# acerbilab/gpyreg

Hardware: AMD Instinct MI355X
Metric: GP-fits/sec (NLL+grad, N=4096 D=10) (higher is better)
Workload: dtype f64

## Files before the change

gpyreg_amd/csrc/gemm.h:

```cpp
#pragma once
#include "common.h"

#include <type_traits>

namespace gpc {

template <typename T>
constexpr int BKT_v = sizeof(T) == 4 ? 32 : 16;
template <typename T>
constexpr bool MM_SWZ = sizeof(T) == 4;
template <typename T>
constexpr int LDQ_v = MM_SWZ<T> ? BKT_v<T> : BKT_v<T> + 1;
constexpr int ldp_of(int BT) { return BT + 16; }
template <typename T>
constexpr int opsz_of(int BT) {
  return BKT_v<T> * (BT + 16) > BT * LDQ_v<T> ? BKT_v<T> * (BT + 16) : BT * LDQ_v<T>;
}

enum { KLO_ZERO = 0, KLO_ROW = 1, KLO_COL = 2 };
enum { KHI_FULL = 0, KHI_ROW = 1, KHI_COL = 2 };

struct GemmArgs {
  const void* A;
  const void* B;
  void* C;
  long long sA, sB, sC;
  int lda, ldb, ldc;
  int M, N, K;
  double alpha;
  int beta;
  int klo, khi, lower_only;
  int tiles_m, tiles_n;
  int flags = 0;
  const unsigned short* rsv = nullptr;
  int* ctr = nullptr;
  int ntiles = 0, batch = 0;
  double* colsq = nullptr;
  const double* ep_w = nullptr;
  long long ep_sw = 0;
  const double* ep_alpha = nullptr;
};
inline int g_gemm_flags = 8 | 16;

template <typename T, bool KM, int BT, int NT>
__device__ __forceinline__ unsigned stage_toff(int ld, int t) {
  constexpr int VEC = MM<T>::VEC;
  if constexpr (!KM) {
    constexpr int TPR = BKT_v<T> / VEC;
    return (unsigned)(t / TPR) * (unsigned)ld + (unsigned)((t % TPR) * VEC);
  } else {
    constexpr int VPR = BT / VEC;
    return (unsigned)(t / VPR) * (unsigned)ld + (unsigned)((t % VPR) * VEC);
  }
}
template <typename T, bool KM, int BT, int NT>
__device__ __forceinline__ size_t stage_pstride(int ld) {
// ... 107 lines not shown
  const int total = gx * gy, per = total >> 3;
  const int L = by * gx + bx;
  if (L < (per << 3)) {
    const int wk = (L & 7) * per + (L >> 3);
    bx = wk % gx;
    by = wk / gx;
  }
}

#ifdef GPC_TILE_TRACE
__device__ unsigned long long g_tile_trace[2][4];
#define TILE_TS(k) do { if (HO && threadIdx.x == 0) { const long long _n = wall_clock64(); atomicAdd(&g_tile_trace[BT == 64][k], (unsigned long long)(_n - _ts)); _ts = _n; } } while (0)
#else
#define TILE_TS(k) do { } while (0)
#endif
template <typename T, bool AKM, bool BKM, int BT, int NW, int HO = 0, int EPI = 0, int BTN = BT>
__device__ __forceinline__ void gemm_tile(const GemmArgs& g, const int bx, const int by, T* __restrict__ smem) {
#ifdef GPC_TILE_TRACE
  long long _ts = wall_clock64();
  if (HO && threadIdx.x == 0) atomicAdd(&g_tile_trace[BT == 64][3], 1ull);
#endif
  using acc_t = typename MM<T>::acc_t;
  using vec_t = typename MM<T>::vec_t;
  constexpr int NT = 64 * NW;
  constexpr int NVA = (BT * BKT_v<T>) / (NT * MM<T>::VEC), NVB = (BTN * BKT_v<T>) / (NT * MM<T>::VEC);
  constexpr int OPSZA = opsz_of<T>(BT), OPSZB = opsz_of<T>(BTN), STG = OPSZA + OPSZB;
  constexpr int WCOLS = NW / 2;
  constexpr int WTM = BT / 2;
  constexpr int WTN = BTN / WCOLS;
  constexpr int MRM = WTM / 16, MRN = WTN / 16;
  static_assert(NVA >= 1 && NVB >= 1 && MRM >= 1 && MRN >= 1, "tile shape");
  const int t = threadIdx.x;
  const int lane = t & 63, w = t >> 6, wr = w / WCOLS, wc = w % WCOLS;

  static_assert(BTN == BT || BT == 2 * BTN, "lower tiles of a rectangular launch: two tile columns per tile row");
  int ti, tj;
  tile_of_bx<BTN == BT>(g.klo, g.khi, g.lower_only, g.tiles_m, g.tiles_n, bx, ti, tj);
  const int m0 = ti * BT, n0 = tj * BTN;
  const int m128 = (m0 / TILE) * TILE, n128 = (n0 / TILE) * TILE;
  int k0 = g.klo == KLO_ROW ? m128 : (g.klo == KLO_COL ? n128 : 0);
  int k1 = g.khi == KHI_ROW ? m128 + TILE : (g.khi == KHI_COL ? n128 + TILE : g.K);
  if (k1 > g.K) k1 = g.K;
  const int nk = (k1 - k0) / BKT_v<T>;

  const T* __restrict__ A = reinterpret_cast<const T*>(g.A) + (size_t)by * g.sA;
  const T* __restrict__ B = reinterpret_cast<const T*>(g.B) + (size_t)by * g.sB;
  T* __restrict__ C = reinterpret_cast<T*>(g.C) + (size_t)by * g.sC;

// ... 38 lines not shown
    };
    constexpr int AUX = HO == 1 ? 16 : 0;
    g2r<T, AKM, BT, NT, AUX>(ra, rsa, ua, psa, toa);
    g2r<T, BKM, BTN, NT, AUX>(rb, rsb, ub, psb, tob);
    r2s<T, AKM, BT, NT>(smem, ra, t);
    r2s<T, BKM, BTN, NT>(smem + OPSZA, rb, t);
    next_slab();
    g2r<T, AKM, BT, NT, AUX>(ra, rsa, ua, psa, toa);
    g2r<T, BKM, BTN, NT, AUX>(rb, rsb, ub, psb, tob);
    __syncthreads();
    TILE_TS(0);

    T af[2][MRM], bf[2][MRN];
    auto load_frags = [&](int set, const T* a_s, const T* b_s, int kk) {
#pragma unroll
      for (int i = 0; i < MRM; ++i) af[set][i] = frag<T, AKM, BT>(a_s, wr * WTM + i * 16, kk, lane);
#pragma unroll
      for (int j = 0; j < MRN; ++j) bf[set][j] = frag<T, BKM, BTN>(b_s, wc * WTN + j * 16, kk, lane);
    };
    auto mfmas = [&](int set) {
#pragma unroll
      for (int i = 0; i < MRM; ++i)
#pragma unroll
        for (int j = 0; j < MRN; ++j) acc[i][j] = MM<T>::mma(af[set][i], bf[set][j], acc[i][j]);
    };
    constexpr int NMEM = NVA + NVB;
    constexpr int PER = (MRM * MRN) / NMEM;
    constexpr int REM = MRM * MRN - PER * NMEM;
    static_assert(PER >= 1, "interleave pattern");
    constexpr int KS = BKT_v<T> / 4;
    static_assert(KS >= 4 && KS % 2 == 0, "fragment sets alternate per k-step and wrap per slab");
    auto slab = [&](auto cur_c, auto wr_c, auto ld_c) {
      constexpr int CUR = decltype(cur_c)::value;
// ... 28 lines not shown
        g2r<T, BKM, BTN, NT, AUX>(rb, rsb, ub, psb, tob);
      }
      if constexpr (WR) load_frags(0, a_n, a_n + OPSZA, 0);
      mfmas(1);
      if constexpr (WR) __builtin_amdgcn_sched_group_barrier(0x100, MRM + MRN, 0);
#pragma unroll
      for (int q = 0; q < NMEM; ++q) {
        __builtin_amdgcn_sched_group_barrier(0x008, PER, 0);
        if constexpr (LD) __builtin_amdgcn_sched_group_barrier(0x020, 1, 0);
      }
      if constexpr (REM > 0) __builtin_amdgcn_sched_group_barrier(0x008, REM, 0);
    };
    using I0 = std::integral_constant<int, 0>;
    using I1 = std::integral_constant<int, 1>;
    load_frags(0, smem, smem + OPSZA, 0);
    int it = 0;
    for (; it + 3 < nk; it += 2) {
      slab(I0{}, std::true_type{}, std::true_type{});
      slab(I1{}, std::true_type{}, std::true_type{});
      if constexpr (TWO_LEVEL) {
#pragma unroll
        for (int i = 0; i < MRM; ++i)
#pragma unroll
          for (int j = 0; j < MRN; ++j) {
            acc2[i][j] += acc[i][j];
            acc[i][j] = acc_t{0, 0, 0, 0};
          }
      }
    }
    slab(I0{}, std::true_type{}, std::false_type{});
    slab(I1{}, std::false_type{}, std::false_type{});
  }

  TILE_TS(1);
  const T alpha = (T)g.alpha;
  if constexpr (EPI == 1) {
    static_assert(NW == 4 && BT == 128 && BTN == BT, "the reduction is laid out for 2 x 2 waves of 64 x 64");
    double cs[MRN];
#pragma unroll
    for (int j = 0; j < MRN; ++j) {
      double sq = 0.0;
#pragma unroll
      for (int i = 0; i < MRM; ++i)
#pragma unroll
        for (int r = 0; r < 4; ++r) {
          double v;
// ... 65 lines not shown
      for (int j = 0; j < MRN; ++j) red[wr * BT + wc * WTN + j * 16 + (lane & 15)] = cs[j];
    }
    __syncthreads();
    if (t < BT) g.colsq[((size_t)by * g.tiles_m + ti) * (size_t)g.N + n0 + t] = red[t] + red[BT + t];
    __syncthreads();
    return;
  }
#pragma unroll
  for (int i = 0; i < MRM; ++i) {
    T old[MRN][4];
    if (g.beta) {
#pragma unroll
      for (int j = 0; j < MRN; ++j)
#pragma unroll
        for (int r = 0; r < 4; ++r) {
          const int row = m0 + wr * WTM + i * 16 + MM<T>::row_of(lane, r);
          const int col = n0 + wc * WTN + j * 16 + (lane & 15);
          if constexpr (HO == 1)
            old[j][r] = __hip_atomic_load(&C[(size_t)row * g.ldc + col], __ATOMIC_RELAXED, __HIP_MEMORY_SCOPE_AGENT);
          else
            old[j][r] = C[(size_t)row * g.ldc + col];
        }
    }
#pragma unroll
    for (int j = 0; j < MRN; ++j)
#pragma unroll
      for (int r = 0; r < 4; ++r) {
        const int row = m0 + wr * WTM + i * 16 + MM<T>::row_of(lane, r);
        const int col = n0 + wc * WTN + j * 16 + (lane & 15);
        T v;
        if constexpr (TWO_LEVEL)
          v = alpha * (acc[i][j][r] + acc2[i][j][r]);
        else
          v = alpha * acc[i][j][r];
        if (g.beta) v += old[j][r];
        if constexpr (HO)
          __hip_atomic_store(&C[(size_t)row * g.ldc + col], v, __ATOMIC_RELAXED, __HIP_MEMORY_SCOPE_AGENT);
        else
          C[(size_t)row * g.ldc + col] = v;
      }
  }
  TILE_TS(2);
}

template <typename T, bool AKM, bool BKM, int BT, int NW, int EPI = 0, int BTN = BT>
__global__ __launch_bounds__(64 * NW, NW / 2) void gemm_kernel(GemmArgs g) {
  __shared__ __attribute__((aligned(16))) T smem[2 * (opsz_of<T>(BT) + opsz_of<T>(BTN))];
  int bx = blockIdx.x, by = blockIdx.y;
  if ((g.flags & 16) && gridDim.y >= 8) {
    xcd_order((int)gridDim.x, (int)gridDim.y, bx, by);
  }
  gemm_tile<T, AKM, BKM, BT, NW, 0, EPI, BTN>(g, bx, by, smem);
}

template <typename T, bool A1, bool B1, bool A2, bool B2, int BT, int NW>
__global__ __launch_bounds__(64 * NW, NW / 2) void gemm_dual_kernel(GemmArgs g1, GemmArgs g2, int n1) {
  __shared__ __attribute__((aligned(16))) T smem[4 * opsz_of<T>(BT)];
  int bx = blockIdx.x, by = blockIdx.y;
  if ((g1.flags & 16) && gridDim.y >= 8) xcd_order((int)gridDim.x, (int)gridDim.y, bx, by);
  if (bx < n1)
    gemm_tile<T, A1, B1, BT, NW>(g1, bx, by, smem);
  else
    gemm_tile<T, A2, B2, BT, NW>(g2, bx - n1, by, smem);
}

template <typename T, bool AKM, bool BKM, int BT, int NW, int EPI = 0>
__global__ __launch_bounds__(64 * NW, NW / 2) void gemm_persist_kernel(GemmArgs g) {
  __shared__ __attribute__((aligned(16))) T smem[4 * opsz_of<T>(BT)];
  __shared__ int next_tile;
  if (g.rsv && cu_reserve_bail(g.rsv, g.ctr)) return;
  if (!(g.flags & 8)) {
    const int total = g.ntiles * g.batch;
    for (;;) {
      if (threadIdx.x == 0) next_tile = atomicAdd(g.ctr, 1);
      __syncthreads();
      const int idx = __builtin_amdgcn_readfirstlane(next_tile);
      __syncthreads();
      if (idx >= total) break;
      gemm_tile<T, AKM, BKM, BT, NW, 0, EPI>(g, idx / g.batch, idx % g.batch, smem);
    }
    return;
  }
  unsigned xcc;
  asm volatile("s_getreg_b32 %0, hwreg(HW_REG_XCC_ID)" : "=s"(xcc));
  const int q0 = (int)(xcc & (NQ - 1));
  const int nclass = g.batch >= NQ ? 1 : NQ / g.batch;
  for (int a = 0; a < NQ; ++a) {
    const int q = (q0 + a) & (NQ - 1);
    int nsq, cls = 0, smp = q;
    if (g.batch >= NQ) {
      nsq = (g.batch - q + NQ - 1) / NQ;
    } else {
      if (q >= g.batch * nclass) continue;
      nsq = 1;
      smp = q % g.batch;
      cls = q / g.batch;
    }
    if (nsq <= 0) continue;
    const int total = ((g.ntiles - cls + nclass - 1) / nclass) * nsq;
    for (;;) {
      if (threadIdx.x == 0) next_tile = atomicAdd(g.ctr + q, 1);
      __syncthreads();
      const int idx = __builtin_amdgcn_readfirstlane(next_tile);
      __syncthreads();
      if (idx >= total) break;
      const int ntq = total / nsq;
      const int sq = idx / ntq, tq = idx - sq * ntq;
      gemm_tile<T, AKM, BKM, BT, NW, 0, EPI>(g, cls + tq * nclass, smp + NQ * sq, smem);
    }
  }
}

inline int queue_nclass(int batch) { return batch >= NQ ? 1 : NQ / batch; }
inline int queue_of(int batch, int nclass, int q, int& cls, int& smp) {
  int nsq;
  cls = 0;
  smp = q;
  if (batch >= NQ) {
    nsq = (batch - q + NQ - 1) / NQ;
  } else {
    if (q >= batch * nclass) return 0;
    nsq = 1;
    smp = q % batch;
    cls = q / batch;
  }
  return nsq;
}
inline int queue_total(int ntiles, int nclass, int cls, int nsq) { return ((ntiles - cls + nclass - 1) / nclass) * nsq; }
inline void queue_item(int total, int nsq, int nclass, int cls, int smp, int idx, int& tile, int& sample) {
  const int ntq = total / nsq;
  const int sq = idx / ntq, tq = idx - sq * ntq;
  tile = cls + tq * nclass;
  sample = smp + NQ * sq;
}
inline void flat_queue_item(int batch, int idx, int& tile, int& sample) {
  tile = idx / batch;
  sample = idx % batch;
}

inline int g_persist_spare = 0;
inline long long g_gemm_launches = 0;
inline int g_block_slots = 512;
template <typename T, int BT, int NW>
inline hipError_t launch_gemm_bt(hipStream_t st, GemmArgs g, bool akm, bool bkm, int batch, int* ctr = nullptr,
                                 const unsigned short* reserve = nullptr) {
  const int tm = g.M / BT, tn = g.N / BT;
  g.tiles_m = tm;
  g.tiles_n = tn;
  g.flags = g_gemm_flags;
  const int ntiles = g.lower_only ? tm * (tm + 1) / 2 : tm * tn;
  if (ntiles <= 0 || batch <= 0) return hipSuccess;
  ++g_gemm_launches;
  g.ntiles = ntiles;
  g.batch = batch;
  g.ctr = ctr;
  const unsigned dyn = 0u;
  const int cap = (BT == 128 ? g_block_slots : 2 * g_block_slots) - g_persist_spare;
  g.rsv = reserve;
  if (ctr && (BT == 128 || reserve) && cap > 0 && ((long long)ntiles * batch > cap || reserve)) {
    dim3 grid(reserve ? (BT == 128 ? cap + 96 : cap) : cap), block(64 * NW);
    if (!akm && !bkm)
      hipLaunchKernelGGL((gemm_persist_kernel<T, false, false, BT, NW>), grid, block, dyn, st, g);
    else if (!akm && bkm)
      hipLaunchKernelGGL((gemm_persist_kernel<T, false, true, BT, NW>), grid, block, dyn, st, g);
    else if (akm && bkm)
      hipLaunchKernelGGL((gemm_persist_kernel<T, true, true, BT, NW>), grid, block, dyn, st, g);
    else
      hipLaunchKernelGGL((gemm_persist_kernel<T, true, false, BT, NW>), grid, block, dyn, st, g);
    return hipGetLastError();
  }
  dim3 grid(ntiles, batch), block(64 * NW);
  if (!akm && !bkm)
    hipLaunchKernelGGL((gemm_kernel<T, false, false, BT, NW>), grid, block, dyn, st, g);
  else if (!akm && bkm)
    hipLaunchKernelGGL((gemm_kernel<T, false, true, BT, NW>), grid, block, dyn, st, g);
  else if (akm && bkm)
    hipLaunchKernelGGL((gemm_kernel<T, true, true, BT, NW>), grid, block, dyn, st, g);
  else
    hipLaunchKernelGGL((gemm_kernel<T, true, false, BT, NW>), grid, block, dyn, st, g);
  return hipGetLastError();
}

#ifdef GPC_EXPERIMENTS
template <typename T>
inline hipError_t launch_gemm_rect(hipStream_t st, GemmArgs g, bool akm, bool bkm, int batch) {
  constexpr int BT = 128, BTN = 64;
// ... 39 lines not shown
  else if (akm && bkm)
    hipLaunchKernelGGL((gemm_kernel<T, true, true, BT, 8>), grid, block, 0, st, g);
  else
    hipLaunchKernelGGL((gemm_kernel<T, true, false, BT, 8>), grid, block, 0, st, g);
  return hipGetLastError();
}
inline int g_rect_min_blocks = 0;
inline int g_rect_mode = 0;

#else
constexpr int g_rect_min_blocks = 0;
#endif

inline int g_small_launch_blocks = 1100;
inline bool g_dual_launch = true;
template <typename T>
inline hipError_t launch_gemm(hipStream_t st, GemmArgs g, bool akm, bool bkm, int batch, int force_bt = 0,
                             int* ctr = nullptr, const unsigned short* reserve = nullptr, int reserved_small_bt = 128) {
  const int tm = g.M / TILE, tn = g.N / TILE;
  const long long blocks128 = (long long)(g.lower_only ? tm * (tm + 1) / 2 : tm * tn) * batch;
  const bool small = force_bt ? (force_bt == 64) : (blocks128 < g_small_launch_blocks);
#ifdef GPC_EXPERIMENTS
  if ((force_bt == 12864 || (!force_bt && small && g_rect_min_blocks > 0 && blocks128 >= g_rect_min_blocks)) && !(reserve && ctr))
    return (g_rect_mode == 1 && force_bt != 12864) ? launch_gemm_w8<T>(st, g, akm, bkm, batch) : launch_gemm_rect<T>(st, g, akm, bkm, batch);
#endif
  if (small && !(reserve && ctr)) return launch_gemm_bt<T, 64, 4>(st, g, akm, bkm, batch);
#ifdef GPC_EXPERIMENTS
  if (small && reserved_small_bt == 64) return launch_gemm_bt<T, 64, 4>(st, g, akm, bkm, batch, ctr, reserve);
#endif
  return launch_gemm_bt<T, 128, 4>(st, g, akm, bkm, batch, ctr, ctr ? reserve : nullptr);
// ... 83 lines not shown
```

gpyreg_amd/csrc/gpcore.hip:

```cpp
#include "../../include/gpcore.h"

#include <algorithm>
#include <atomic>
#include <chrono>
#include <cmath>
#include <cstdlib>
#include <cstring>
#include <memory>
#include <mutex>

#include "blas1.h"
#include "block_append.h"
#include "common.h"
#include "covfun.h"
#include "cv.h"
#include "cvgrad.h"
#include "draw.h"
#include "gemm.h"
#include "gradpost.h"
#include "hess.h"
#include "hypgrad.h"
#include "nll_hess.h"
#include "leaf.h"
#include "lookahead.h"
// ... 3987 lines not shown
              {rb, cb, p.ldb, p.off_b, p.s_b, p.size_b, true},
              {p.M, p.N, p.ldc, p.off_c, p.s_c, p.size_c, false}};
  for (const Op& o : ops) {
    if (o.ld < o.cols || o.off < 0 || o.stride < 0 || o.size <= 0 || o.size > CAP || o.ld > CAP || o.stride > CAP)
      return "leading dimension below the extent, or a negative / oversized offset, stride or allocation";
    const long long span = (o.rows - 1) * o.ld + o.cols;
    if (o.off + (batch - 1) * o.stride + span > o.size) return "an operand reaches past its allocation";
    if (o.staged && (o.ld % vec || o.off % vec || o.stride % vec))
      return "lda, ldb and the offsets and strides of A and B must be multiples of the 16-byte vector";
    if (!o.staged && batch > 1 && o.stride < span) return "the C blocks of two samples overlap";
  }
  return nullptr;
}

template <typename T>
int debug_gemm_form_impl(gpc_ctx* c, int form, int tile, int batch, int flags, int block_slots,
                         const gpc_gemm_product* const* prods, int nprod, const double* ep_w, long long ep_sw,
                         const double* ep_alpha, double* colsq, int* counters, int* available) {
  HookMem mem;
  GemmGlobalsGuard guard;
  if (flags >= 0) gpc::g_gemm_flags = flags;
  if (block_slots > 0) {
    gpc::g_block_slots = block_slots;
    gpc::g_persist_spare = 0;
  }
  const unsigned short* rsv = nullptr;
  if (form == GPC_FORM_PERSIST_RESERVED) {
    rsv = ctx_reserve_tbl(c);
    if (!rsv) {
      *available = 0;
      return 0;
// ... 25 lines not shown
    a.C = dC[i] + p.off_c;
    a.sA = p.s_a;
    a.sB = p.s_b;
    a.sC = p.s_c;
    a.lda = p.lda;
    a.ldb = p.ldb;
    a.ldc = p.ldc;
    a.M = p.M;
    a.N = p.N;
    a.K = p.K;
    a.alpha = p.alpha;
    a.beta = p.beta;
    a.klo = p.klo;
    a.khi = p.khi;
    a.lower_only = p.lower_only ? 1 : 0;
  }
  int* ctr = nullptr;
  HIPCHK(c, mem.get(reinterpret_cast<void**>(&ctr), CTR_STRIDE * sizeof(int)));
  HIPCHK(c, hipMemsetAsync(ctr, 0, CTR_STRIDE * sizeof(int), c->st));
  const gpc_gemm_product& p0 = *prods[0];
  const size_t ncolsq = (size_t)batch * (p0.M / TILE) * p0.N;
  double* dcolsq = nullptr;
  if (form == GPC_FORM_COLSQ || form == GPC_FORM_WSQ) {
    HIPCHK(c, mem.get(reinterpret_cast<void**>(&dcolsq), ncolsq * sizeof(double)));
    HIPCHK(c, hipMemsetAsync(dcolsq, 0xff, ncolsq * sizeof(double), c->st));
    g[0].colsq = dcolsq;
  }
  if (form == GPC_FORM_WSQ) {
    double *dw = nullptr, *da = nullptr;
    const size_t nw = (size_t)(batch - 1) * ep_sw + p0.M;
// ... 2454 lines not shown
#ifdef GPC_EXPERIMENTS
constexpr int IS_EXPERIMENTS_BUILD = 1;
#else
constexpr int IS_EXPERIMENTS_BUILD = 0;
#endif
int clamp_to(int lo, int hi, int v) { return std::max(lo, std::min(hi, v)); }
int tile_multiple(int v) { return std::max(TILE, (v / TILE) * TILE); }
int engine_choice(int v) { return v == 1 || v == 2 ? v : 0; }
#define GPC_GET(expr) [](gpc_ctx* c) -> int { (void)c; return (int)(expr); }
#define GPC_SET(stmt) [](gpc_ctx* c, int v) -> int { (void)c; stmt; return 0; }
#define GPC_COUNTER(field) GPC_GET(c->field & 0x7fffffff), nullptr
const Option OPTIONS[] = {
    {"groups", GPC_GET(c->groups), GPC_SET(c->groups = clamp_to(1, gpc_ctx::MAXG, v))},
    {"small_blocks", GPC_GET(gpc::g_small_launch_blocks), GPC_SET(gpc::g_small_launch_blocks = v)},
    {"dual_launch", GPC_GET(gpc::g_dual_launch ? 1 : 0), GPC_SET(gpc::g_dual_launch = v != 0)},
    {"leaf", GPC_GET(gpc::g_leaf_version), GPC_SET(gpc::g_leaf_version = v == 3 ? 3 : 5)},
    {"defer_min", GPC_GET(c->defer_min), GPC_SET(c->defer_min = v)},
    {"defer_reserve", GPC_GET(c->defer_reserve), [](gpc_ctx* c, int v) -> int { return c->defer_reserve = v, build_reserve_table(c); }},
    {"leaf_fault", nullptr, GPC_SET(gpc::g_leaf_fault = v != 0)},
    {"nll_block", GPC_GET(c->nll_block), GPC_SET(c->nll_block = v < 0 ? -1 : (v == 0 ? 0 : tile_multiple(v)))},
    {"solves_beside_lauum", GPC_GET(c->solves_beside_lauum), GPC_SET(c->solves_beside_lauum = v != 0)},
    {"stable", GPC_GET(c->stable), GPC_SET(c->stable = v != 0)},
    {"small_path", GPC_GET(c->small_path), GPC_SET(c->small_path = v != 0)},
    {"check_queues", GPC_GET(c->check_queues), GPC_SET(c->check_queues = v != 0)},
    {"small_poll", GPC_GET(c->small_poll), GPC_SET(c->small_poll = v != 0)},
    {"small_timing", GPC_GET(c->small_timing), GPC_SET(c->small_timing = v != 0)},
    {"small_polled", GPC_COUNTER(small_polled)},
    {"small_synced", GPC_COUNTER(small_synced)},
    {"hess_contract_us", GPC_COUNTER(hess_contract_us)},
    {"nll_hess_gram_us", GPC_COUNTER(nll_hess_gram_us)},
// ... 206 lines not shown
    for (int by = 0; by < batch; ++by)
      for (int bx = 0; bx < ntiles; ++bx) {
        int x = bx, y = by;
        if ((flags & 16) && batch >= 8) xcd_order(ntiles, batch, x, y);
        xcd_items[2 * (by * ntiles + bx)] = x;
        xcd_items[2 * (by * ntiles + bx) + 1] = y;
      }
  }
  return 0;
}

int gpc_debug_gemm_form(gpc_ctx* c, int dtype, int form, int tile, int batch, int flags, int block_slots,
                        const gpc_gemm_product* p1, const gpc_gemm_product* p2, const double* ep_w, long long ep_sw,
                        const double* ep_alpha, double* colsq, int* counters, int* available) {
  if (!c) return -2;
  if (!p1 || !counters || !available || batch <= 0 || batch > 64 || form < GPC_FORM_PLAIN || form > GPC_FORM_WSQ ||
      (tile != 64 && tile != 128) || (dtype != GPC_F64 && dtype != GPC_F32) || flags > 31 || block_slots > 4096)
    FAIL(c, "gpc_debug_gemm_form: bad arguments");
  const int vec = dtype == GPC_F64 ? 2 : 4;
  const gpc_gemm_product* prods[2] = {p1, p2};
  const int nprod = form == GPC_FORM_DUAL ? 2 : 1;
  if (nprod == 2 && !p2) FAIL(c, "gpc_debug_gemm_form: the dual form takes two products");
  for (int i = 0; i < nprod; ++i)
    if (const char* e = form_product_error(*prods[i], batch, vec)) {
      c->err = std::string("gpc_debug_gemm_form: ") + e;
      return -2;
    }
  if (form == GPC_FORM_DUAL && (p1->a_kmajor || p1->b_kmajor || p2->a_kmajor || !p2->b_kmajor))
    FAIL(c, "gpc_debug_gemm_form: the dual launch is m-major x m-major beside m-major x k-major");
  if (form == GPC_FORM_COLSQ && (p1->a_kmajor || !p1->b_kmajor || p1->lower_only || !colsq))
    FAIL(c, "gpc_debug_gemm_form: colsq is m-major x k-major over all tiles and needs the colsq output");
  if (form == GPC_FORM_WSQ && (!p1->a_kmajor || !p1->b_kmajor || p1->lower_only || !colsq || !ep_w || !ep_alpha ||
                               (batch > 1 && ep_sw != 0 && ep_sw < p1->M) || ep_sw < 0 || ep_sw > (1ll << 27)))
    FAIL(c, "gpc_debug_gemm_form: wsq is k-major x k-major over all tiles and needs colsq, ep_w, ep_alpha");
  HIPCHK(c, hipSetDevice(c->device));
  return dtype == GPC_F64 ? debug_gemm_form_impl<double>(c, form, tile, batch, flags, block_slots, prods, nprod, ep_w, ep_sw,
                                                         ep_alpha, colsq, counters, available)
                          : debug_gemm_form_impl<float>(c, form, tile, batch, flags, block_slots, prods, nprod, ep_w, ep_sw,
                                                        ep_alpha, colsq, counters, available);
}

int gpc_debug_leaf(gpc_ctx* c, int dtype, const double* A, double* L, double* W, double* logdet, int* info) {
  return gpc_debug_factor(c, dtype, TILE, A, L, W, nullptr, logdet, info);
}

int gpc_debug_factor(gpc_ctx* c, int dtype, int n, const double* A, double* L, double* W, double* Ainv,
                     double* logdet, int* info) {
  if (!c) return -2;
  if (!A || n <= 0) FAIL(c, "gpc_debug_factor: bad arguments");
  HIPCHK(c, hipSetDevice(c->device));
  return dtype == GPC_F64 ? debug_factor_impl<double>(c, n, A, L, W, Ainv, logdet, info)
                          : debug_factor_impl<float>(c, n, A, L, W, Ainv, logdet, info);
}
// ... 305 lines not shown
```

gpyreg_amd/csrc/plan.h:

```cpp
#pragma once
#include "blas1.h"
#include "gemm.h"
#include "leaf.h"

#include <algorithm>

namespace gpc {

#ifdef GPC_EXPERIMENTS
struct PlanRecorder {
  struct Op {
    int kind;
    GemmArgs g;
    bool akm, bkm;
    int off;
  };
  std::vector<Op> ops;
  bool unsupported = false;
};
#endif

template <typename T>
struct Factor {
#ifdef GPC_EXPERIMENTS
// ... 20 lines not shown
  const unsigned short* reserve = nullptr;
  struct QueueCheck {
    int* slot;
    int ntiles, batch;
  };
  std::vector<QueueCheck>* qlog = nullptr;
#ifdef GPC_EXPERIMENTS
  bool reserve_all = false;
  int reserve_min = 64;
  int reserved_small_bt = 128;
#else
  static constexpr bool reserve_all = false;
  static constexpr int reserve_min = 64, reserved_small_bt = 128;
#endif
  bool dual_launch = g_dual_launch;
  bool stable = false;
  hipEvent_t ev_tail = nullptr;
  int tail_row0 = 1 << 30;
  void need_rows(int hi) {
    if (ev_tail && hi > tail_row0) {
      chk(hipStreamWaitEvent(st, ev_tail, 0));
      ev_tail = nullptr;
    }
  }
  double flops = 0;
  int launches = 0;
  hipError_t err = hipSuccess;

  T* blk(T* base, int r, int c) const { return base + (size_t)r * npad + c; }

// ... 10 lines not shown
    g.M = M;
    g.N = N;
    g.K = K;
    g.alpha = alpha;
    g.beta = beta;
    g.klo = klo;
    g.khi = khi;
    g.lower_only = lower;
    g.tiles_n = N / TILE;
    flops += gemm_flops(g, batch);
    return g;
  }

  void gemm(T* C, long long sC, const T* Aop, long long sAop, const T* Bop, long long sBop, int M,
            int N, int K, bool akm, bool bkm, double alpha, int beta, int klo, int khi, int lower,
            hipStream_t on = nullptr, const unsigned short* rsv = nullptr) {
    GemmArgs g;
    g.A = Aop;
    g.B = Bop;
    g.C = C;
    g.sA = sAop;
    g.sB = sBop;
    g.sC = sC;
    g.lda = g.ldb = g.ldc = npad;
    g.M = M;
    g.N = N;
    g.K = K;
    g.alpha = alpha;
    g.beta = beta;
    g.klo = klo;
    g.khi = khi;
    g.lower_only = lower;
    g.tiles_n = N / TILE;
    flops += gemm_flops(g, batch);
    ++launches;
#ifdef GPC_EXPERIMENTS
    if (rec) {
      rec->ops.push_back({0, g, akm, bkm, 0});
      return;
    }
#endif
    int* slot = nullptr;
    const long long tm = M / TILE, tn = N / TILE;
    const long long blocks128 = (lower ? tm * (tm + 1) / 2 : tm * tn) * batch;
    if (!rsv && reserve_all && reserve && blocks128 >= reserve_min) rsv = reserve;
    const bool persistent = rsv || (blocks128 >= g_small_launch_blocks && blocks128 > g_block_slots - g_persist_spare);
    if (persistent && ctr && ctr_used + CTR_STRIDE <= ctr_cap) {
// ... 22 lines not shown
      }
#endif
      need_rows(off + TILE);
      launch_leaf<T>(st, batch, blk(A, off, off), sA, npad, blk(W, off, off), sW, npad, off, logdet, info,
                     std::max(0, std::min(TILE, nvalid - off)), stable);
      flops += (2.0 / 3.0) * TILE * (double)TILE * TILE * batch;
      ++launches;
      return;
    }
    const int q = n / TILE;
    const int n1 = (q / 2) * TILE, n2 = n - n1;
    const int o1 = off, o2 = off + n1;
    potrf_inv(o1, n1, true, keep_L);
    need_rows(o2 + n2);
    gemm(blk(Tm, o2, o1), sT, blk(A, o2, o1), sA, blk(W, o1, o1), sW, n2, n1, n1, false, false, 1.0,
         0, KLO_ZERO, KHI_COL, 0);
    if (stable) {
      gemm(blk(A, o2, o1), sA, blk(Tm, o2, o1), sT, blk(A, o1, o1), sA, n2, n1, n1, false, false, -1.0, 1, KLO_ZERO,
           KHI_COL, 0);
      gemm(blk(Tm, o2, o1), sT, blk(A, o2, o1), sA, blk(W, o1, o1), sW, n2, n1, n1, false, false, 1.0, 1, KLO_ZERO,
           KHI_COL, 0);
    }
    const bool defer = need_inv && side && defer_min > 0 && n >= defer_min && ev_used + 2 <= nev;
    bool u_done = false;
    {
      GemmArgs gs = make_args(blk(A, o2, o2), sA, blk(Tm, o2, o1), sT, blk(Tm, o2, o1), sT, n2, n2, n1, -1.0, 1,
                              KLO_ZERO, KHI_FULL, 1);
      const long long syrk_tiles = (long long)(n2 / TILE) * (n2 / TILE + 1) / 2 * batch;
      if (need_inv && !defer && dual_launch && !rec && gemm_is_small(gs, batch) && !(reserve_all && syrk_tiles >= reserve_min)) {
        GemmArgs gu = make_args(blk(A, o2, o1), sA, blk(Tm, o2, o1), sT, blk(W, o1, o1), sW, n2, n1, n1, 1.0, 0,
                                KLO_COL, KHI_FULL, 0);
// ... 7 lines not shown
        }
      }
      if (!u_done) {
        flops -= gemm_flops(gs, batch);
        gemm(blk(A, o2, o2), sA, blk(Tm, o2, o1), sT, blk(Tm, o2, o1), sT, n2, n2, n1, false, false, -1.0, 1,
             KLO_ZERO, KHI_FULL, 1);
      }
    }
    hipEvent_t ev_join = nullptr;
    if (defer) {
      hipEvent_t ev_fork = evs[ev_used++];
      ev_join = evs[ev_used++];
      chk(hipEventRecord(ev_fork, st));
      chk(hipStreamWaitEvent(side, ev_fork, 0));
      gemm(blk(A, o2, o1), sA, blk(Tm, o2, o1), sT, blk(W, o1, o1), sW, n2, n1, n1, false, true, 1.0, 0,
           KLO_COL, KHI_FULL, 0, side, reserve);
      chk(hipEventRecord(ev_join, side));
    }
    potrf_inv(o2, n2, need_inv, keep_L);
    if (need_inv) {
      if (defer)
        chk(hipStreamWaitEvent(st, ev_join, 0));
      else if (!u_done)
        gemm(blk(A, o2, o1), sA, blk(Tm, o2, o1), sT, blk(W, o1, o1), sW, n2, n1, n1, false, true, 1.0, 0,
             KLO_COL, KHI_FULL, 0);
      gemm(blk(W, o2, o1), sW, blk(W, o2, o2), sW, blk(A, o2, o1), sA, n2, n1, n2, false, true, -1.0,
           0, KLO_ZERO, KHI_ROW, 0);
    }
#ifdef GPC_EXPERIMENTS
    if (keep_L && rec) rec->unsupported = true;
#endif
    if (keep_L && !rec) {
      dim3 grid((n1 + 64 * MM<T>::VEC - 1) / (64 * MM<T>::VEC), n2 / 32, batch), block(64, 4);
      hipLaunchKernelGGL((rect_copy_kernel<T>), grid, block, 0, st, (const T*)blk(Tm, o2, o1), sT, npad,
                         blk(A, o2, o1), sA, npad, n2, n1);
      ++launches;
    }
  }

  int nll_block = 0;

  void trsm_nll(int r0, int m, int c0, int n) {
// ... 114 lines not shown
        hipLaunchKernelGGL((trmv_kernel<T>), dim3(n / 4, batch), dim3(256), 0, st, (const T*)W, sW, npad,
                           (const double*)r, npad, z, off);
      ++launches;
      return;
    }
    const int q = n / TILE;
    const int n1 = (q / 2) * TILE, n2 = n - n1;
    forward_solve(off, n1, true, r, z);
    hipLaunchKernelGGL((gemv_sub_kernel<T>), dim3(n2 / 4, batch), dim3(256), 0, st, (const T*)Tm, sT, npad,
                       (const double*)z, r, npad, off + n1, off, n1);
    ++launches;
    forward_solve(off + n1, n2, need_inv, r, z);
  }

  void lauum(T* out, long long sOut) {
    gemm(out, sOut, W, sW, W, sW, npad, npad, npad, true, true, 1.0, 0, KLO_ROW, KHI_FULL, 1);
  }
};

}
```

Before: 844.5.

## Skip zero MFMAs inside triangular diagonal blocks of fp64 128-tile GEMMs

Adds a TRI template mode to the fp64 128-tile GEMM. In the k-slabs that cross a triangular operand's diagonal block, each wave issues only the MFMAs for sub-tile rows or columns that can be nonzero. The wave-to-subtile mapping is interleaved so the skipped work is spread evenly across waves. The mode is wired into the trsm, inverse-update and lauum calls, with a runtime toggle that defaults to on. In exchange it adds kernel instantiations, runtime branches in the slab loop, and a changed fragment layout that may cost register or scheduling efficiency.

```diff
diff --git a/gpyreg_amd/csrc/gemm.h b/gpyreg_amd/csrc/gemm.h
--- a/gpyreg_amd/csrc/gemm.h
+++ b/gpyreg_amd/csrc/gemm.h
@@ -19,6 +19,7 @@
 
 enum { KLO_ZERO = 0, KLO_ROW = 1, KLO_COL = 2 };
 enum { KHI_FULL = 0, KHI_ROW = 1, KHI_COL = 2 };
+enum { TRI_NONE = 0, TRI_A_FIRST = 1, TRI_B_FIRST = 2, TRI_B_LAST = 3, TRI_A_LAST = 4 };
 
 struct GemmArgs {
   const void* A;
@@ -32,6 +33,7 @@
   int klo, khi, lower_only;
   int tiles_m, tiles_n;
   int flags = 0;
+  int tri = 0;
   const unsigned short* rsv = nullptr;
   int* ctr = nullptr;
   int ntiles = 0, batch = 0;
@@ -40,6 +42,7 @@
   long long ep_sw = 0;
   const double* ep_alpha = nullptr;
 };
+static_assert(sizeof(GemmArgs) == 168, "tri fills the hole behind flags: the kernel arguments keep their offsets and size");
 inline int g_gemm_flags = 8 | 16;
 
 template <typename T, bool KM, int BT, int NT>
@@ -177,7 +180,7 @@
 #else
 #define TILE_TS(k) do { } while (0)
 #endif
-template <typename T, bool AKM, bool BKM, int BT, int NW, int HO = 0, int EPI = 0, int BTN = BT>
+template <typename T, bool AKM, bool BKM, int BT, int NW, int HO = 0, int EPI = 0, int BTN = BT, int TRI = 0>
 __device__ __forceinline__ void gemm_tile(const GemmArgs& g, const int bx, const int by, T* __restrict__ smem) {
 #ifdef GPC_TILE_TRACE
   long long _ts = wall_clock64();
@@ -193,8 +196,16 @@
   constexpr int WTN = BTN / WCOLS;
   constexpr int MRM = WTM / 16, MRN = WTN / 16;
   static_assert(NVA >= 1 && NVB >= 1 && MRM >= 1 && MRN >= 1, "tile shape");
+  static_assert(TRI == 0 || (sizeof(T) == 8 && BT == 128 && BTN == BT && NW == 4 && HO == 0 && EPI == 0),
+                "triangular blocks: the fp64 128-tile of 2 x 2 waves, stored");
+  static_assert(TRI == 0 || (TRI == TRI_A_FIRST && AKM) || (TRI == TRI_B_FIRST && BKM) || (TRI == TRI_B_LAST && !BKM) ||
+                    (TRI == TRI_A_LAST && !AKM), "the orientation of the triangular operand");
   const int t = threadIdx.x;
   const int lane = t & 63, w = t >> 6, wr = w / WCOLS, wc = w % WCOLS;
+#define GPC_WROW(i) (TRI ? (wr + 2 * (i)) * 16 : wr * WTM + (i) * 16)
+#define GPC_WCOL(j) (TRI ? (wc + 2 * (j)) * 16 : wc * WTN + (j) * 16)
+#define GPC_ROW(o, i) (TRI ? (o) + (wr + 2 * (i)) * 16 : (o) + wr * WTM + (i) * 16)
+#define GPC_COL(o, j) (TRI ? (o) + (wc + 2 * (j)) * 16 : (o) + wc * WTN + (j) * 16)
 
   static_assert(BTN == BT || BT == 2 * BTN, "lower tiles of a rectangular launch: two tile columns per tile row");
   int ti, tj;
@@ -263,9 +274,9 @@
     T af[2][MRM], bf[2][MRN];
     auto load_frags = [&](int set, const T* a_s, const T* b_s, int kk) {
 #pragma unroll
-      for (int i = 0; i < MRM; ++i) af[set][i] = frag<T, AKM, BT>(a_s, wr * WTM + i * 16, kk, lane);
-#pragma unroll
-      for (int j = 0; j < MRN; ++j) bf[set][j] = frag<T, BKM, BTN>(b_s, wc * WTN + j * 16, kk, lane);
+      for (int i = 0; i < MRM; ++i) af[set][i] = frag<T, AKM, BT>(a_s, GPC_WROW(i), kk, lane);
+#pragma unroll
+      for (int j = 0; j < MRN; ++j) bf[set][j] = frag<T, BKM, BTN>(b_s, GPC_WCOL(j), kk, lane);
     };
     auto mfmas = [&](int set) {
 #pragma unroll
@@ -324,22 +335,103 @@
     using I0 = std::integral_constant<int, 0>;
     using I1 = std::integral_constant<int, 1>;
     load_frags(0, smem, smem + OPSZA, 0);
-    int it = 0;
-    for (; it + 3 < nk; it += 2) {
-      slab(I0{}, std::true_type{}, std::true_type{});
-      slab(I1{}, std::true_type{}, std::true_type{});
-      if constexpr (TWO_LEVEL) {
-#pragma unroll
-        for (int i = 0; i < MRM; ++i)
-#pragma unroll
-          for (int j = 0; j < MRN; ++j) {
-            acc2[i][j] += acc[i][j];
-            acc[i][j] = acc_t{0, 0, 0, 0};
+    if constexpr (TRI != 0) {
+      constexpr bool ON_A = TRI == TRI_A_FIRST || TRI == TRI_A_LAST, FIRST = TRI == TRI_A_FIRST || TRI == TRI_B_FIRST;
+      const int wq = __builtin_amdgcn_readfirstlane(ON_A ? wr : wc);
+      auto mfmas_tri = [&](int set, int lo, int hi) {
+        if constexpr (ON_A) {
+#pragma unroll
+          for (int i = 0; i < MRM; ++i)
+            if (i >= lo && i < hi) {
+#pragma unroll
+              for (int j = 0; j < MRN; ++j) acc[i][j] = MM<T>::mma(af[set][i], bf[set][j], acc[i][j]);
+            }
+        } else {
+#pragma unroll
+          for (int j = 0; j < MRN; ++j)
+            if (j >= lo && j < hi) {
+#pragma unroll
+              for (int i = 0; i < MRM; ++i) acc[i][j] = MM<T>::mma(af[set][i], bf[set][j], acc[i][j]);
+            }
+        }
+      };
+      auto slab_tri = [&](auto cur_c, const bool WR, const bool LD, const int lo, const int hi) {
+        constexpr int CUR = decltype(cur_c)::value;
+        const T* a_s = smem + CUR * STG;
+        const T* b_s = a_s + OPSZA;
+        T* a_n = smem + (CUR ^ 1) * STG;
+#pragma unroll
+        for (int ks = 0; ks < KS - 2; ++ks) {
+          load_frags((ks + 1) & 1, a_s, b_s, 4 * (ks + 1));
+          mfmas_tri(ks & 1, lo, hi);
+        }
+        load_frags(1, a_s, b_s, 4 * (KS - 1));
+        if (WR) {
+          r2s<T, AKM, BT, NT>(a_n, ra, t);
+          r2s<T, BKM, BTN, NT>(a_n + OPSZA, rb, t);
+        }
+        mfmas_tri(0, lo, hi);
+        __syncthreads();
+        if (LD) {
+          next_slab();
+          g2r<T, AKM, BT, NT, AUX>(ra, rsa, ua, psa, toa);
+          g2r<T, BKM, BTN, NT, AUX>(rb, rsb, ub, psb, tob);
+        }
+        if (WR) load_frags(0, a_n, a_n + OPSZA, 0);
+        mfmas_tri(1, lo, hi);
+      };
+      auto tri_pair = [&](const int s, const bool more) {
+        int lo[2], hi[2];
+#pragma unroll
+        for (int e = 0; e < 2; ++e) {
+          const int d = s + e - wq;
+          lo[e] = FIRST ? 0 : (d > 0 ? (d + 1) >> 1 : 0);
+          hi[e] = FIRST ? (d >= 0 ? (d >> 1) + 1 : 0) : 4;
+        }
+        slab_tri(I0{}, true, more, lo[0], hi[0]);
+        slab_tri(I1{}, more, more, lo[1], hi[1]);
+      };
+      constexpr int NTRI = TILE / BKT_v<T>;
+      static_assert(MRM == 4 && MRN == 4 && NTRI == 8, "live prefixes and suffixes of four tile-rows over eight slabs");
+      if constexpr (FIRST) {
+#pragma unroll 1
+        for (int s = 0; s < NTRI; s += 2) tri_pair(s, s + 2 < nk);
+        if (nk > NTRI) {
+#pragma unroll 1
+          for (int it = NTRI; it + 3 < nk; it += 2) {
+            slab(I0{}, std::true_type{}, std::true_type{});
+            slab(I1{}, std::true_type{}, std::true_type{});
           }
-      }
-    }
-    slab(I0{}, std::true_type{}, std::false_type{});
-    slab(I1{}, std::false_type{}, std::false_type{});
+          slab(I0{}, std::true_type{}, std::false_type{});
+          slab(I1{}, std::false_type{}, std::false_type{});
+        }
+      } else {
+#pragma unroll 1
+        for (int it = 0; it < nk - NTRI; it += 2) {
+          slab(I0{}, std::true_type{}, std::true_type{});
+          slab(I1{}, std::true_type{}, std::true_type{});
+        }
+#pragma unroll 1
+        for (int s = 0; s < NTRI; s += 2) tri_pair(s, s + 2 < NTRI);
+      }
+    } else {
+      int it = 0;
+      for (; it + 3 < nk; it += 2) {
+        slab(I0{}, std::true_type{}, std::true_type{});
+        slab(I1{}, std::true_type{}, std::true_type{});
+        if constexpr (TWO_LEVEL) {
+#pragma unroll
+          for (int i = 0; i < MRM; ++i)
+#pragma unroll
+            for (int j = 0; j < MRN; ++j) {
+              acc2[i][j] += acc[i][j];
+              acc[i][j] = acc_t{0, 0, 0, 0};
+            }
+        }
+      }
+      slab(I0{}, std::true_type{}, std::false_type{});
+      slab(I1{}, std::false_type{}, std::false_type{});
+    }
   }
 
   TILE_TS(1);
@@ -435,8 +527,8 @@
       for (int j = 0; j < MRN; ++j)
 #pragma unroll
         for (int r = 0; r < 4; ++r) {
-          const int row = m0 + wr * WTM + i * 16 + MM<T>::row_of(lane, r);
-          const int col = n0 + wc * WTN + j * 16 + (lane & 15);
+          const int row = GPC_ROW(m0, i) + MM<T>::row_of(lane, r);
+          const int col = GPC_COL(n0, j) + (lane & 15);
           if constexpr (HO == 1)
             old[j][r] = __hip_atomic_load(&C[(size_t)row * g.ldc + col], __ATOMIC_RELAXED, __HIP_MEMORY_SCOPE_AGENT);
           else
@@ -447,8 +539,8 @@
     for (int j = 0; j < MRN; ++j)
 #pragma unroll
       for (int r = 0; r < 4; ++r) {
-        const int row = m0 + wr * WTM + i * 16 + MM<T>::row_of(lane, r);
-        const int col = n0 + wc * WTN + j * 16 + (lane & 15);
+        const int row = GPC_ROW(m0, i) + MM<T>::row_of(lane, r);
+        const int col = GPC_COL(n0, j) + (lane & 15);
         T v;
         if constexpr (TWO_LEVEL)
           v = alpha * (acc[i][j][r] + acc2[i][j][r]);
@@ -462,16 +554,20 @@
       }
   }
   TILE_TS(2);
-}
-
-template <typename T, bool AKM, bool BKM, int BT, int NW, int EPI = 0, int BTN = BT>
+#undef GPC_WROW
+#undef GPC_WCOL
+#undef GPC_ROW
+#undef GPC_COL
+}
+
+template <typename T, bool AKM, bool BKM, int BT, int NW, int EPI = 0, int BTN = BT, int TRI = 0>
 __global__ __launch_bounds__(64 * NW, NW / 2) void gemm_kernel(GemmArgs g) {
   __shared__ __attribute__((aligned(16))) T smem[2 * (opsz_of<T>(BT) + opsz_of<T>(BTN))];
   int bx = blockIdx.x, by = blockIdx.y;
   if ((g.flags & 16) && gridDim.y >= 8) {
     xcd_order((int)gridDim.x, (int)gridDim.y, bx, by);
   }
-  gemm_tile<T, AKM, BKM, BT, NW, 0, EPI, BTN>(g, bx, by, smem);
+  gemm_tile<T, AKM, BKM, BT, NW, 0, EPI, BTN, TRI>(g, bx, by, smem);
 }
 
 template <typename T, bool A1, bool B1, bool A2, bool B2, int BT, int NW>
@@ -485,7 +581,7 @@
     gemm_tile<T, A2, B2, BT, NW>(g2, bx - n1, by, smem);
 }
 
-template <typename T, bool AKM, bool BKM, int BT, int NW, int EPI = 0>
+template <typename T, bool AKM, bool BKM, int BT, int NW, int EPI = 0, int TRI = 0>
 __global__ __launch_bounds__(64 * NW, NW / 2) void gemm_persist_kernel(GemmArgs g) {
   __shared__ __attribute__((aligned(16))) T smem[4 * opsz_of<T>(BT)];
   __shared__ int next_tile;
@@ -498,7 +594,7 @@
       const int idx = __builtin_amdgcn_readfirstlane(next_tile);
       __syncthreads();
       if (idx >= total) break;
-      gemm_tile<T, AKM, BKM, BT, NW, 0, EPI>(g, idx / g.batch, idx % g.batch, smem);
+      gemm_tile<T, AKM, BKM, BT, NW, 0, EPI, BT, TRI>(g, idx / g.batch, idx % g.batch, smem);
     }
     return;
   }
@@ -527,7 +623,7 @@
       if (idx >= total) break;
       const int ntq = total / nsq;
       const int sq = idx / ntq, tq = idx - sq * ntq;
-      gemm_tile<T, AKM, BKM, BT, NW, 0, EPI>(g, cls + tq * nclass, smp + NQ * sq, smem);
+      gemm_tile<T, AKM, BKM, BT, NW, 0, EPI, BT, TRI>(g, cls + tq * nclass, smp + NQ * sq, smem);
     }
   }
 }
@@ -557,6 +653,18 @@
 inline void flat_queue_item(int batch, int idx, int& tile, int& sample) {
   tile = idx / batch;
   sample = idx % batch;
+}
+
+template <typename T, int BT>
+inline int gemm_tri_of(const GemmArgs& g, bool akm, bool bkm) {
+  if (sizeof(T) != 8 || BT != 128) return TRI_NONE;
+  switch (g.tri) {
+    case TRI_A_FIRST: return akm && bkm && g.klo == KLO_ROW && g.khi == KHI_FULL && g.K >= g.M ? TRI_A_FIRST : TRI_NONE;
+    case TRI_B_FIRST: return !akm && bkm && g.klo == KLO_COL && g.khi == KHI_FULL && g.K >= g.N ? TRI_B_FIRST : TRI_NONE;
+    case TRI_B_LAST: return !akm && !bkm && g.klo == KLO_ZERO && g.khi == KHI_COL && g.K >= g.N ? TRI_B_LAST : TRI_NONE;
+    case TRI_A_LAST: return !akm && bkm && g.klo == KLO_ZERO && g.khi == KHI_ROW && g.K >= g.M ? TRI_A_LAST : TRI_NONE;
+    default: return TRI_NONE;
+  }
 }
 
 inline int g_persist_spare = 0;
@@ -578,8 +686,20 @@
   const unsigned dyn = 0u;
   const int cap = (BT == 128 ? g_block_slots : 2 * g_block_slots) - g_persist_spare;
   g.rsv = reserve;
+  const int tri = gemm_tri_of<T, BT>(g, akm, bkm);
   if (ctr && (BT == 128 || reserve) && cap > 0 && ((long long)ntiles * batch > cap || reserve)) {
     dim3 grid(reserve ? (BT == 128 ? cap + 96 : cap) : cap), block(64 * NW);
+    if constexpr (sizeof(T) == 8 && BT == 128 && NW == 4) {
+      if (tri == TRI_A_FIRST)
+        hipLaunchKernelGGL((gemm_persist_kernel<T, true, true, BT, NW, 0, TRI_A_FIRST>), grid, block, dyn, st, g);
+      else if (tri == TRI_B_FIRST)
+        hipLaunchKernelGGL((gemm_persist_kernel<T, false, true, BT, NW, 0, TRI_B_FIRST>), grid, block, dyn, st, g);
+      else if (tri == TRI_B_LAST)
+        hipLaunchKernelGGL((gemm_persist_kernel<T, false, false, BT, NW, 0, TRI_B_LAST>), grid, block, dyn, st, g);
+      else if (tri == TRI_A_LAST)
+        hipLaunchKernelGGL((gemm_persist_kernel<T, false, true, BT, NW, 0, TRI_A_LAST>), grid, block, dyn, st, g);
+      if (tri) return hipGetLastError();
+    }
     if (!akm && !bkm)
       hipLaunchKernelGGL((gemm_persist_kernel<T, false, false, BT, NW>), grid, block, dyn, st, g);
     else if (!akm && bkm)
@@ -591,6 +711,17 @@
     return hipGetLastError();
   }
   dim3 grid(ntiles, batch), block(64 * NW);
+  if constexpr (sizeof(T) == 8 && BT == 128 && NW == 4) {
+    if (tri == TRI_A_FIRST)
+      hipLaunchKernelGGL((gemm_kernel<T, true, true, BT, NW, 0, BT, TRI_A_FIRST>), grid, block, dyn, st, g);
+    else if (tri == TRI_B_FIRST)
+      hipLaunchKernelGGL((gemm_kernel<T, false, true, BT, NW, 0, BT, TRI_B_FIRST>), grid, block, dyn, st, g);
+    else if (tri == TRI_B_LAST)
+      hipLaunchKernelGGL((gemm_kernel<T, false, false, BT, NW, 0, BT, TRI_B_LAST>), grid, block, dyn, st, g);
+    else if (tri == TRI_A_LAST)
+      hipLaunchKernelGGL((gemm_kernel<T, false, true, BT, NW, 0, BT, TRI_A_LAST>), grid, block, dyn, st, g);
+    if (tri) return hipGetLastError();
+  }
   if (!akm && !bkm)
     hipLaunchKernelGGL((gemm_kernel<T, false, false, BT, NW>), grid, block, dyn, st, g);
   else if (!akm && bkm)
@@ -660,6 +791,7 @@
 
 inline int g_small_launch_blocks = 1100;
 inline bool g_dual_launch = true;
+inline bool g_tri_skip = true;
 template <typename T>
 inline hipError_t launch_gemm(hipStream_t st, GemmArgs g, bool akm, bool bkm, int batch, int force_bt = 0,
                              int* ctr = nullptr, const unsigned short* reserve = nullptr, int reserved_small_bt = 128) {
diff --git a/gpyreg_amd/csrc/gpcore.hip b/gpyreg_amd/csrc/gpcore.hip
--- a/gpyreg_amd/csrc/gpcore.hip
+++ b/gpyreg_amd/csrc/gpcore.hip
@@ -4025,7 +4025,7 @@
 }
 
 template <typename T>
-int debug_gemm_form_impl(gpc_ctx* c, int form, int tile, int batch, int flags, int block_slots,
+int debug_gemm_form_impl(gpc_ctx* c, int form, int tile, int batch, int flags, int tri, int block_slots,
                          const gpc_gemm_product* const* prods, int nprod, const double* ep_w, long long ep_sw,
                          const double* ep_alpha, double* colsq, int* counters, int* available) {
   HookMem mem;
@@ -4081,6 +4081,7 @@
     a.klo = p.klo;
     a.khi = p.khi;
     a.lower_only = p.lower_only ? 1 : 0;
+    a.tri = tri;
   }
   int* ctr = nullptr;
   HIPCHK(c, mem.get(reinterpret_cast<void**>(&ctr), CTR_STRIDE * sizeof(int)));
@@ -6565,6 +6566,7 @@
     {"groups", GPC_GET(c->groups), GPC_SET(c->groups = clamp_to(1, gpc_ctx::MAXG, v))},
     {"small_blocks", GPC_GET(gpc::g_small_launch_blocks), GPC_SET(gpc::g_small_launch_blocks = v)},
     {"dual_launch", GPC_GET(gpc::g_dual_launch ? 1 : 0), GPC_SET(gpc::g_dual_launch = v != 0)},
+    {"tri_skip", GPC_GET(gpc::g_tri_skip ? 1 : 0), GPC_SET(gpc::g_tri_skip = v != 0)},
     {"leaf", GPC_GET(gpc::g_leaf_version), GPC_SET(gpc::g_leaf_version = v == 3 ? 3 : 5)},
     {"defer_min", GPC_GET(c->defer_min), GPC_SET(c->defer_min = v)},
     {"defer_reserve", GPC_GET(c->defer_reserve), [](gpc_ctx* c, int v) -> int { return c->defer_reserve = v, build_reserve_table(c); }},
@@ -6801,6 +6803,9 @@
                         const gpc_gemm_product* p1, const gpc_gemm_product* p2, const double* ep_w, long long ep_sw,
                         const double* ep_alpha, double* colsq, int* counters, int* available) {
   if (!c) return -2;
+  const int tri = flags >= 0 ? (flags >> 8) & 7 : 0;
+  if (flags >= 0) flags &= ~0x700;
+  if (tri > gpc::TRI_A_LAST) FAIL(c, "gpc_debug_gemm_form: bad arguments");
   if (!p1 || !counters || !available || batch <= 0 || batch > 64 || form < GPC_FORM_PLAIN || form > GPC_FORM_WSQ ||
       (tile != 64 && tile != 128) || (dtype != GPC_F64 && dtype != GPC_F32) || flags > 31 || block_slots > 4096)
     FAIL(c, "gpc_debug_gemm_form: bad arguments");
@@ -6821,9 +6826,9 @@
                                (batch > 1 && ep_sw != 0 && ep_sw < p1->M) || ep_sw < 0 || ep_sw > (1ll << 27)))
     FAIL(c, "gpc_debug_gemm_form: wsq is k-major x k-major over all tiles and needs colsq, ep_w, ep_alpha");
   HIPCHK(c, hipSetDevice(c->device));
-  return dtype == GPC_F64 ? debug_gemm_form_impl<double>(c, form, tile, batch, flags, block_slots, prods, nprod, ep_w, ep_sw,
+  return dtype == GPC_F64 ? debug_gemm_form_impl<double>(c, form, tile, batch, flags, tri, block_slots, prods, nprod, ep_w, ep_sw,
                                                          ep_alpha, colsq, counters, available)
-                          : debug_gemm_form_impl<float>(c, form, tile, batch, flags, block_slots, prods, nprod, ep_w, ep_sw,
+                          : debug_gemm_form_impl<float>(c, form, tile, batch, flags, tri, block_slots, prods, nprod, ep_w, ep_sw,
                                                         ep_alpha, colsq, counters, available);
 }
 
diff --git a/gpyreg_amd/csrc/plan.h b/gpyreg_amd/csrc/plan.h
--- a/gpyreg_amd/csrc/plan.h
+++ b/gpyreg_amd/csrc/plan.h
@@ -58,6 +58,7 @@
   static constexpr int reserve_min = 64, reserved_small_bt = 128;
 #endif
   bool dual_launch = g_dual_launch;
+  bool tri_skip = g_tri_skip;
   bool stable = false;
   hipEvent_t ev_tail = nullptr;
   int tail_row0 = 1 << 30;
@@ -98,7 +99,7 @@
 
   void gemm(T* C, long long sC, const T* Aop, long long sAop, const T* Bop, long long sBop, int M,
             int N, int K, bool akm, bool bkm, double alpha, int beta, int klo, int khi, int lower,
-            hipStream_t on = nullptr, const unsigned short* rsv = nullptr) {
+            hipStream_t on = nullptr, const unsigned short* rsv = nullptr, int tri = TRI_NONE) {
     GemmArgs g;
     g.A = Aop;
     g.B = Bop;
@@ -115,6 +116,7 @@
     g.klo = klo;
     g.khi = khi;
     g.lower_only = lower;
+    g.tri = tri_skip ? tri : TRI_NONE;
     g.tiles_n = N / TILE;
     flops += gemm_flops(g, batch);
     ++launches;
@@ -167,7 +169,7 @@
     potrf_inv(o1, n1, true, keep_L);
     need_rows(o2 + n2);
     gemm(blk(Tm, o2, o1), sT, blk(A, o2, o1), sA, blk(W, o1, o1), sW, n2, n1, n1, false, false, 1.0,
-         0, KLO_ZERO, KHI_COL, 0);
+         0, KLO_ZERO, KHI_COL, 0, nullptr, nullptr, TRI_B_LAST);
     if (stable) {
       gemm(blk(A, o2, o1), sA, blk(Tm, o2, o1), sT, blk(A, o1, o1), sA, n2, n1, n1, false, false, -1.0, 1, KLO_ZERO,
            KHI_COL, 0);
@@ -205,7 +207,7 @@
       chk(hipEventRecord(ev_fork, st));
       chk(hipStreamWaitEvent(side, ev_fork, 0));
       gemm(blk(A, o2, o1), sA, blk(Tm, o2, o1), sT, blk(W, o1, o1), sW, n2, n1, n1, false, true, 1.0, 0,
-           KLO_COL, KHI_FULL, 0, side, reserve);
+           KLO_COL, KHI_FULL, 0, side, reserve, TRI_B_FIRST);
       chk(hipEventRecord(ev_join, side));
     }
     potrf_inv(o2, n2, need_inv, keep_L);
@@ -214,9 +216,9 @@
         chk(hipStreamWaitEvent(st, ev_join, 0));
       else if (!u_done)
         gemm(blk(A, o2, o1), sA, blk(Tm, o2, o1), sT, blk(W, o1, o1), sW, n2, n1, n1, false, true, 1.0, 0,
-             KLO_COL, KHI_FULL, 0);
+             KLO_COL, KHI_FULL, 0, nullptr, nullptr, TRI_B_FIRST);
       gemm(blk(W, o2, o1), sW, blk(W, o2, o2), sW, blk(A, o2, o1), sA, n2, n1, n2, false, true, -1.0,
-           0, KLO_ZERO, KHI_ROW, 0);
+           0, KLO_ZERO, KHI_ROW, 0, nullptr, nullptr, TRI_A_LAST);
     }
 #ifdef GPC_EXPERIMENTS
     if (keep_L && rec) rec->unsupported = true;
@@ -361,7 +363,8 @@
   }
 
   void lauum(T* out, long long sOut) {
-    gemm(out, sOut, W, sW, W, sW, npad, npad, npad, true, true, 1.0, 0, KLO_ROW, KHI_FULL, 1);
+    gemm(out, sOut, W, sW, W, sW, npad, npad, npad, true, true, 1.0, 0, KLO_ROW, KHI_FULL, 1, nullptr, nullptr,
+         TRI_A_FIRST);
   }
 };
 
```

After: 846.6 (median of 2 runs). No clear change (+0.2%).
